# ushariRanasinghe/G2VLM

Hardware: AMD Instinct MI355X
Metric: views/sec (multi-view recon, G2VLM-2B-MoT) (higher is better)
Workload: dtype bf16; 1 GPU; C3: 8-view 518x518 reconstruction, full depth (24 DINO + 28 MoT + 15 decoder blocks), 1 scene per GPU; Lq=10968, Lk=10976, parallelism=replicas x1

## Files before the change

g2vlm_amd/csrc/gemm.hip:

```cpp
#include "common.h"
#include "g2vlm_hip.h"
#include "gemm_internal.h"

namespace {

constexpr int BM = 128, BN = 128, BK = 64;
constexpr int TILE_BYTES = BM * BK * 2;

struct GemmGroup {
  const __bf16* A;
  const __bf16* W;
  const __bf16* bias;
  void* C;
  const void* res;
  const float* gamma;
  int M;
  int tile_start;
};

struct GemmArgs {
  GemmGroup g[2];
  int ngroups, N, K, lda, ldc, ldres, tiles_n, flags, sm, sn, g0_tiles;
};

__device__ __forceinline__ u32x4 ld_chunk(const __bf16* base, int row, int ld, int k, int K) {
  u32x4 z = {0, 0, 0, 0};
  if (k >= K) return z;
  return *reinterpret_cast<const u32x4*>(base + (size_t)row * ld + k);
}

template <int EPI>
__global__ __launch_bounds__(256, 2) void gemm_bf16_kernel(GemmArgs a) {
  __shared__ __attribute__((aligned(16))) char smem[2 * TILE_BYTES];
  char* sA = smem;
  char* sB = smem + TILE_BYTES;

  int bid = blockIdx.x;
  int gi = (a.ngroups > 1 && bid >= a.g[1].tile_start) ? 1 : 0;
  const GemmGroup g = a.g[gi];
  int t = bid - g.tile_start;
  int tm, tn;
  if (a.sm > 1 && gi == 0) {
    const int nt = a.g0_tiles;
    int xcd = t & 7, qn = nt >> 3, rn = nt & 7;
    t = (xcd < rn ? xcd * (qn + 1) : rn * (qn + 1) + (xcd - rn) * qn) + (t >> 3);
    const int tiles_m = (g.M + BM - 1) / BM;
    const int row_sz = a.sm * a.tiles_n;
    int sup_m = t / row_sz, r = t - sup_m * row_sz;
    int h = min(a.sm, tiles_m - sup_m * a.sm);
    int full_w = a.sn * h;
    int sup_n = r / full_w, p = r - sup_n * full_w;
    int width = min(a.sn, a.tiles_n - sup_n * a.sn);
// ... 86 lines not shown
      for (int jp = 0; jp < 2; ++jp) {
        int oc = ((n0 + wn * 64) >> 1) + jp * 16 + cl;
        if (oc >= (N >> 1)) continue;
#pragma unroll
        for (int r = 0; r < 4; ++r) {
          int gm = rbase + i * 16 + r;
          if (gm >= M) continue;
          float gt = bfround(acc[i][2 * jp][r]);
          float up = bfround(acc[i][2 * jp + 1][r]);
          float s = bfround(siluf_fast_(gt));
          C[(size_t)gm * a.ldc + oc] = f2bf(s * up);
        }
      }
    return;
  } else {
#pragma unroll
    for (int j = 0; j < 4; ++j) {
      int gn = n0 + wn * 64 + j * 16 + cl;
      if (gn >= N) continue;
      float bv = g.bias ? bf2f(g.bias[gn]) : 0.f;
      float gam = (EPI == G2V_EPI_RES_F32 && g.gamma) ? g.gamma[gn] : 1.f;
#pragma unroll
      for (int i = 0; i < 4; ++i)
#pragma unroll
        for (int r = 0; r < 4; ++r) {
          int gm = rbase + i * 16 + r;
          if (gm >= M) continue;
          float v = bfround(acc[i][j][r] + bv);
          size_t o = (size_t)gm * a.ldc + gn;
          if constexpr (EPI == G2V_EPI_BF16) {
            reinterpret_cast<__bf16*>(g.C)[o] = f2bf(v);
          } else if constexpr (EPI == G2V_EPI_GELU) {
            reinterpret_cast<__bf16*>(g.C)[o] = f2bf(gelu_erf(v));
          } else if constexpr (EPI == G2V_EPI_QUICKGELU) {
            float u = bfround(1.702f * v);
            float s = bfround(sigmoidf_(u));
            reinterpret_cast<__bf16*>(g.C)[o] = f2bf(v * s);
          } else if constexpr (EPI == G2V_EPI_RES_F32) {
            if (g.gamma) {
              v = __fmul_rn(v, gam);
              if (a.flags & G2V_GEMM_GAMMA_ROUND_BF16) v = bfround(v);
            }
            float rv = g.res ? reinterpret_cast<const float*>(g.res)[(size_t)gm * a.ldres + gn] : 0.f;
            reinterpret_cast<float*>(g.C)[o] = __fadd_rn(rv, v);
          } else if constexpr (EPI == G2V_EPI_RES_BF16) {
            float rv = bf2f(reinterpret_cast<const __bf16*>(g.res)[(size_t)gm * a.ldres + gn]);
            reinterpret_cast<__bf16*>(g.C)[o] = f2bf(rv + v);
          }
        }
    }
  }
}

constexpr int FBK = 16, FLD = 144;

struct GemmF32Args {
  const float* A; const float* W; const float* bias; float* C; const float* res;
  int M, N, K, lda, ldc, ldres, tiles_n, relu;
};

__global__ __launch_bounds__(256, 2) void gemm_f32_kernel(GemmF32Args a) {
  __shared__ __attribute__((aligned(16))) float sA[FBK * FLD];
  __shared__ __attribute__((aligned(16))) float sB[FBK * FLD];
  int tm = blockIdx.x / a.tiles_n, tn = blockIdx.x - tm * a.tiles_n;
  int m0 = tm * 128, n0 = tn * 128;
  const int tid = threadIdx.x, lane = tid & 63, w = tid >> 6, wm = w >> 1, wn = w & 1;
  int srow[2], sk[2], ar[2], br[2];
#pragma unroll
  for (int i = 0; i < 2; ++i) {
    int id = tid + 256 * i;
    srow[i] = id >> 2; sk[i] = (id & 3) * 4;
    ar[i] = min(m0 + srow[i], a.M - 1);
    br[i] = min(n0 + srow[i], a.N - 1);
  }
  f32x4 ra[2], rb[2];
  auto ld4 = [&](const float* base, int row, int ld, int k) -> f32x4 {
    f32x4 v = {0.f, 0.f, 0.f, 0.f};
    const float* p = base + (size_t)row * ld + k;
    if (k + 3 < a.K) v = *reinterpret_cast<const f32x4*>(p);
    else { for (int e = 0; e < 4; ++e) if (k + e < a.K) v[e] = p[e]; }
    return v;
  };
  auto stage_load = [&](int k0) {
#pragma unroll
    for (int i = 0; i < 2; ++i) { ra[i] = ld4(a.A, ar[i], a.lda, k0 + sk[i]); rb[i] = ld4(a.W, br[i], a.K, k0 + sk[i]); }
  };
  auto stage_write = [&]() {
#pragma unroll
    for (int i = 0; i < 2; ++i)
#pragma unroll
      for (int e = 0; e < 4; ++e) { sA[(sk[i] + e) * FLD + srow[i]] = ra[i][e]; sB[(sk[i] + e) * FLD + srow[i]] = rb[i][e]; }
  };
  f32x4 acc[4][4];
#pragma unroll
  for (int i = 0; i < 4; ++i)
#pragma unroll
    for (int j = 0; j < 4; ++j) acc[i][j] = f32x4{0.f, 0.f, 0.f, 0.f};
  const int nk = (a.K + FBK - 1) / FBK;
  stage_load(0); stage_write(); __syncthreads();
  for (int kt = 0; kt < nk; ++kt) {
    if (kt + 1 < nk) stage_load((kt + 1) * FBK);
#pragma unroll
    for (int ks = 0; ks < 4; ++ks) {
      float fa[4], fb[4];
      int kq = ks * 4 + (lane >> 4);
#pragma unroll
      for (int i = 0; i < 4; ++i) {
        fa[i] = sA[kq * FLD + wm * 64 + i * 16 + (lane & 15)];
        fb[i] = sB[kq * FLD + wn * 64 + i * 16 + (lane & 15)];
      }
#pragma unroll
      for (int i = 0; i < 4; ++i)
#pragma unroll
        for (int j = 0; j < 4; ++j) acc[i][j] = __builtin_amdgcn_mfma_f32_16x16x4f32(fa[i], fb[j], acc[i][j], 0, 0, 0);
    }
    __syncthreads();
    if (kt + 1 < nk) { stage_write(); __syncthreads(); }
  }
  const int rbase = m0 + wm * 64 + ((lane >> 4) << 2), cl = lane & 15;
#pragma unroll
  for (int j = 0; j < 4; ++j) {
    int gn = n0 + wn * 64 + j * 16 + cl;
    if (gn >= a.N) continue;
    float bv = a.bias ? a.bias[gn] : 0.f;
#pragma unroll
    for (int i = 0; i < 4; ++i)
#pragma unroll
      for (int r = 0; r < 4; ++r) {
        int gm = rbase + i * 16 + r;
        if (gm >= a.M) continue;
        float v = acc[i][j][r] + bv;
        if (a.relu) v = fmaxf(v, 0.f);
        if (a.res) v = a.res[(size_t)gm * a.ldres + gn] + v;
        a.C[(size_t)gm * a.ldc + gn] = v;
      }
  }
}

template <int EPI>
int launch_bf16(const GemmArgs& a, int total_tiles, hipStream_t s) {
  hipLaunchKernelGGL(gemm_bf16_kernel<EPI>, dim3(total_tiles), dim3(256), 0, s, a);
  G2V_CHECK_LAUNCH();
  return G2V_OK;
}

}

enum { FORM_128 = 1, FORM_BIG = 2, FORM_8P = 3, FORM_4W = 4, FORM_SKINNY = 5 };

static int gemm_route(const g2v_gemm_desc* d, int32_t r[4]) {
  if (!d || d->ngroups < 1 || d->ngroups > 2 || d->N <= 0 || d->K <= 0 || (d->K & 7) || (d->lda & 7)) return G2V_ERR_ARG;
  if (d->epilogue == G2V_EPI_SWIGLU && (d->N & 31)) return G2V_ERR_ARG;
  for (int i = 0; i < d->ngroups; ++i)
    if (d->g[i].M < 0 || !d->g[i].W || !d->g[i].C || (d->g[i].M > 0 && !d->g[i].A)) return G2V_ERR_ARG;
  const bool res_bf16 = d->epilogue == G2V_EPI_RES_BF16;
  r[2] = r[3] = 1;
  const int force = d->flags & (G2V_GEMM_FORCE_SMALL_TILE | G2V_GEMM_FORCE_BIG_TILE | G2V_GEMM_FORCE_8P);
  if (force == 0 && g2v_gemm_skinny_eligible(d)) {
    int M = 0;
    for (int i = 0; i < d->ngroups; ++i) {
      if (res_bf16 && d->g[i].M > 0 && !d->g[i].res) return G2V_ERR_ARG;
      if (d->g[i].M > 0) M = d->g[i].M;
    }
    r[0] = FORM_SKINNY; r[1] = M <= 16 ? 16 : (M <= 32 ? 32 : 64);
    g2v_gemm_skinny_split(d, M, &r[2], &r[3]);
    return G2V_OK;
  }
  if (g2v_gemm_8p_supported(d) && (force == G2V_GEMM_FORCE_8P || (force == 0 && g2v_gemm_8p_preferred(d)))) {
    if (res_bf16)
      for (int i = 0; i < d->ngroups; ++i) if (!d->g[i].res) return G2V_ERR_ARG;
    r[0] = g2v_gemm_8p_four_waves(d) ? FORM_4W : FORM_8P; r[1] = g2v_gemm_8p_height(d);
    return G2V_OK;
  }
  if (!(d->flags & G2V_GEMM_FORCE_SMALL_TILE) && ((d->flags & G2V_GEMM_FORCE_BIG_TILE) ? (d->K % 64 == 0 && d->N % 256 == 0) : g2v_gemm_big_eligible(d))) {
    r[0] = FORM_BIG; r[1] = g2v_gemm_big_height(d);
    return G2V_OK;
  }
  if (res_bf16)
    for (int i = 0; i < d->ngroups; ++i) if (!d->g[i].res) return G2V_ERR_ARG;
  r[0] = FORM_128; r[1] = BM;
  return G2V_OK;
}

extern "C" int g2v_gemm_route(const g2v_gemm_desc* d, int32_t out[4]) {
  if (!out) return G2V_ERR_ARG;
  return gemm_route(d, out);
}

extern "C" int g2v_gemm_bf16(const g2v_gemm_desc* d, void* stream) {
  int32_t r[4];
  const int rc = gemm_route(d, r);
  if (rc != G2V_OK) return rc;
  if (r[0] == FORM_SKINNY) return g2v_gemm_skinny_launch(d, (hipStream_t)stream);
  if (r[0] == FORM_8P || r[0] == FORM_4W) return g2v_gemm_8p_launch(d, (hipStream_t)stream);
  if (r[0] == FORM_BIG) return g2v_gemm_big_launch(d, (hipStream_t)stream);
  GemmArgs a;
  a.ngroups = d->ngroups; a.N = d->N; a.K = d->K; a.lda = d->lda; a.ldc = d->ldc; a.ldres = d->ldres;
  a.tiles_n = (d->N + BN - 1) / BN; a.flags = d->flags;
  int total = 0;
  for (int i = 0; i < 2; ++i) {
    const g2v_gemm_group& s = d->g[i < d->ngroups ? i : 0];
    GemmGroup& g = a.g[i];
    g.A = (const __bf16*)s.A; g.W = (const __bf16*)s.W; g.bias = (const __bf16*)s.bias; g.C = s.C;
    g.res = s.res; g.gamma = (const float*)s.gamma; g.M = s.M; g.tile_start = total;
    if (i < d->ngroups) total += ((s.M + BM - 1) / BM) * a.tiles_n;
  }
  a.sm = 1; a.sn = 1;
  a.sn = a.tiles_n < 12 ? a.tiles_n : 12; a.sm = 96 / a.sn > 1 ? 96 / a.sn : 1;
  if (a.ngroups == 2 && a.g[1].M == 0) a.ngroups = 1;
  if (a.ngroups == 2 && a.g[0].M == 0) { a.g[0] = a.g[1]; a.g[0].tile_start = 0; a.ngroups = 1; }
  if (total == 0) return G2V_OK;
  a.g0_tiles = a.ngroups > 1 ? a.g[1].tile_start : total;
  hipStream_t s = (hipStream_t)stream;
  switch (d->epilogue) {
    case G2V_EPI_BF16: return launch_bf16<G2V_EPI_BF16>(a, total, s);
    case G2V_EPI_GELU: return launch_bf16<G2V_EPI_GELU>(a, total, s);
    case G2V_EPI_QUICKGELU: return launch_bf16<G2V_EPI_QUICKGELU>(a, total, s);
    case G2V_EPI_SWIGLU: return launch_bf16<G2V_EPI_SWIGLU>(a, total, s);
    case G2V_EPI_RES_F32: return launch_bf16<G2V_EPI_RES_F32>(a, total, s);
    case G2V_EPI_RES_BF16: return launch_bf16<G2V_EPI_RES_BF16>(a, total, s);
    default: return G2V_ERR_ARG;
  }
}

extern "C" int g2v_gemm_f32(const void* A, const void* W, const void* bias, void* C, const void* res,
                            int M, int N, int K, int lda, int ldc, int ldres, int relu, void* stream) {
  if (!A || !W || !C || M < 0 || N <= 0 || K <= 0 || (lda & 3) || (K & 3)) return G2V_ERR_ARG;
  if (M == 0) return G2V_OK;
  GemmF32Args a{(const float*)A, (const float*)W, (const float*)bias, (float*)C, (const float*)res,
                M, N, K, lda, ldc, ldres, (N + 127) / 128, relu};
  int tiles = ((M + 127) / 128) * a.tiles_n;
  hipLaunchKernelGGL(gemm_f32_kernel, dim3(tiles), dim3(256), 0, (hipStream_t)stream, a);
  G2V_CHECK_LAUNCH();
  return G2V_OK;
}
```

g2vlm_amd/engine.py:

```python
import math
import os

import torch

from . import hip
from .decode import Decode, KVCache, linear_names, weight_key


def rope2d_tables(D, seq_len, base=100.0):
    inv_freq = 1.0 / (base ** (torch.arange(0, D, 2).float() / D))
    t = torch.arange(seq_len, dtype=inv_freq.dtype)
    freqs = torch.einsum("i,j->ij", t, inv_freq).to(torch.bfloat16)
    freqs = torch.cat((freqs, freqs), dim=-1)
    return freqs.cos(), freqs.sin()


def attn_tile_rows(windows, Hq):
    long_kv = sum(w[3] for w in windows if w[0] == windows[0][0]) >= 2048 and max(w[1] for w in windows) >= 2048
    tall = False
    if not long_kv:
        pad = lambda t: sum((w[1] + t - 1) // t * t for w in windows) / max(1, sum(w[1] for w in windows))
        items = sum((w[1] + 255) // 256 for w in windows) * Hq
        tall = items >= 512 and pad(256) <= 1.12 * pad(128)
    return 256 if (long_kv or tall) else 128
# ... 393 lines not shown
                hp.rope2d(cq, 0, nh, D, cos, sin, pos, P)
                hp.flash_attn(cq, ckv[:, :C], ckv[:, C:], ao, cross_plan, nh, nh, D)
                hp.linear(ao, w[p + "cproj.w"], w[p + "cproj.b"], hp.EPI_RES_F32, out=x, res=x)
                n_mlp = "norm3"
            else:
                n_mlp = "norm2"
            hp.layernorm(x, w[p + n_mlp + ".w"], w[p + n_mlp + ".b"], 1e-6, out=h)
            hp.linear(h, w[p + "mlp.fc1.w"], w[p + "mlp.fc1.b"], hp.EPI_GELU, out=mid)
            hp.linear(mid, w[p + "mlp.fc2.w"], w[p + "mlp.fc2.b"], hp.EPI_RES_F32, out=x, res=x)
        return hp.linear(hp.cast_bf16(x), w[name + ".out.w"], w[name + ".out.b"])

    def decoders_and_heads(self, hidden, context, N, gh, gw, H, W):
        P = gh * gw
        mode = "0" if torch.cuda.is_current_stream_capturing() else os.environ.get("G2V_HEADS_OVERLAP", "2")
        if mode == "0":
            point_hidden = self.decoder("point_decoder", hidden, N, gh, gw)
            camera_hidden = self.decoder("camera_decoder", hidden, N, gh, gw)
            global_hidden = self.decoder("global_points_decoder", hidden, N, gh, gw, context=context)
            points, local, poses, glob = self.heads(point_hidden, camera_hidden, global_hidden, N, H, W)
            return point_hidden, camera_hidden, global_hidden, points, local, poses, glob
        cur = torch.cuda.current_stream()
        side = self.side_stream(cur)
        if mode == "1":
            camera_hidden = self.decoder("camera_decoder", hidden, N, gh, gw)
            side.wait_stream(cur)
            with torch.cuda.stream(side):
                poses = self.camera_poses(camera_hidden, N, P)
            point_hidden = self.decoder("point_decoder", hidden, N, gh, gw)
            side.wait_stream(cur)
            with torch.cuda.stream(side):
                points, local = self.point_maps_local(point_hidden, poses, N, H, W)
            global_hidden = self.decoder("global_points_decoder", hidden, N, gh, gw, context=context)
            cur.wait_stream(side)
            glob = self.point_maps_global(global_hidden, N, H, W)
            return point_hidden, camera_hidden, global_hidden, points, local, poses, glob
        side.wait_stream(cur)
        with torch.cuda.stream(side):
            global_hidden = self.decoder("global_points_decoder", hidden, N, gh, gw, context=context)
            glob = self.point_maps_global(global_hidden, N, H, W)
        camera_hidden = self.decoder("camera_decoder", hidden, N, gh, gw)
        poses = self.camera_poses(camera_hidden, N, P)
        point_hidden = self.decoder("point_decoder", hidden, N, gh, gw)
        points, local = self.point_maps_local(point_hidden, poses, N, H, W)
        cur.wait_stream(side)
        return point_hidden, camera_hidden, global_hidden, points, local, poses, glob

    def side_stream(self, cur):
        key = cur.cuda_stream
        if key not in self._side_streams:
            self._side_streams[key] = torch.cuda.Stream(device=self.dev)
        return self._side_streams[key]

    def conf_head(self, conf_hidden, N, H, W):
        cf = hip.gemm_f32(hip.cast_f32(conf_hidden), self.w["conf_head.w"], self.w["conf_head.b"])
        return hip.pixel_shuffle(cf, N, H, W, 1, self.patch)

    def camera_poses(self, camera_hidden, N, P):
        w, hp = self.w, hip
        feat = hp.cast_f32(camera_hidden)
        for i in range(2):
            t = hp.gemm_f32(feat, w[f"cam.res{i}.1.w"], w[f"cam.res{i}.1.b"], relu=True)
            t = hp.gemm_f32(t, w[f"cam.res{i}.2.w"], w[f"cam.res{i}.2.b"], relu=True)
            feat = hp.gemm_f32(t, w[f"cam.res{i}.3.w"], w[f"cam.res{i}.3.b"], relu=True, res=feat)
        return hp.camera_tail(feat, N, P, w["cam.mlp0.w"], w["cam.mlp0.b"], w["cam.mlp1.w"], w["cam.mlp1.b"],
                              w["cam.fc_t.w"], w["cam.fc_t.b"], w["cam.fc_rot.w"], w["cam.fc_rot.b"])

    def point_maps(self, point_hidden, global_hidden, poses, N, H, W):
        points, local = self.point_maps_local(point_hidden, poses, N, H, W)
        return points, local, self.point_maps_global(global_hidden, N, H, W)

    def point_maps_local(self, point_hidden, poses, N, H, W):
        w, hp = self.w, hip
        pf = hp.gemm_f32(hp.cast_f32(point_hidden), w["point_head.w"], w["point_head.b"])
        local, points = hp.pts_epilogue(pf, N, H, W, 1, poses, patch=self.patch)
        return points, local

    def point_maps_global(self, global_hidden, N, H, W):
        w, hp = self.w, hip
        gf = hp.gemm_f32(hp.cast_f32(global_hidden), w["global_point_head.w"], w["global_point_head.b"])
        glob, _ = hp.pts_epilogue(gf, N, H, W, 0, patch=self.patch)
        return glob

    def heads(self, point_hidden, camera_hidden, global_hidden, N, H, W):
        poses = self.camera_poses(camera_hidden, N, (H // self.patch) * (W // self.patch))
        points, local, glob = self.point_maps(point_hidden, global_hidden, poses, N, H, W)
        return points, local, poses, glob

    def vit_forward(self, pixel_values, grid_thw, cos, sin, num_layers=None, n_images=1):
        w, hp = self.w, hip
        V = self.dims["vit"]
        C, nh = V["embed"], V["heads"]
        D = C // nh
        T = pixel_values.shape[0]
        t, gh, gw = grid_thw
        t = t * n_images
        assert pixel_values.shape[1] == w["vit.patch.w"].shape[1] and T == t * gh * gw
        x = hp.linear(pixel_values if pixel_values.dtype == torch.bfloat16 else hp.cast_bf16(pixel_values), w["vit.patch.w"], None)
        plan = self.plan(tuple((i * gh * gw, gh * gw, i * gh * gw, gh * gw, False) for i in range(t)), nh)
        h = torch.empty((T, C), dtype=torch.bfloat16, device=self.dev)
        qkv = torch.empty((T, 3 * C), dtype=torch.bfloat16, device=self.dev)
        ao = torch.empty((T, C), dtype=torch.bfloat16, device=self.dev)
        mid = torch.empty((T, int(C * V["mlp_ratio"])), dtype=torch.bfloat16, device=self.dev)
        for i in range(V["depth"] if num_layers is None else num_layers):
            p = f"V{i}."
            hp.layernorm(x, w[p + "norm1.w"], w[p + "norm1.b"], 1e-6, out=h)
            hp.linear(h, w[p + "attn.qkv.w"], w[p + "attn.qkv.b"], out=qkv)
            hp.rope_vision(qkv, 2 * nh, D, cos, sin)
            hp.flash_attn(qkv[:, :C], qkv[:, C:2 * C], qkv[:, 2 * C:], ao, plan, nh, nh, D)
            hp.linear(ao, w[p + "attn.proj.w"], w[p + "attn.proj.b"], hp.EPI_RES_BF16, out=x, res=x)
            hp.layernorm(x, w[p + "norm2.w"], w[p + "norm2.b"], 1e-6, out=h)
            hp.linear(h, w[p + "mlp.fc1.w"], w[p + "mlp.fc1.b"], hp.EPI_QUICKGELU, out=mid)
            hp.linear(mid, w[p + "mlp.fc2.w"], w[p + "mlp.fc2.b"], hp.EPI_RES_BF16, out=x, res=x)
        hp.layernorm(x, w["vit.ln_q.w"], w["vit.ln_q.b"], 1e-6, out=h)
        m = hp.linear(h.view(T // 4, 4 * C), w["vit.m0.w"], w["vit.m0.b"], hp.EPI_GELU)
        return hp.linear(m, w["vit.m2.w"], w["vit.m2.b"])
```

g2vlm_amd/hip.py:

```python
import ctypes as C
import os
import threading

import torch

_HERE = os.path.dirname(os.path.abspath(__file__))
LIB_PATH = os.environ.get("G2V_LIB_PATH") or os.path.join(_HERE, "lib", "libg2vlm_hip.so")

EPI_BF16, EPI_GELU, EPI_QUICKGELU, EPI_SWIGLU, EPI_RES_F32, EPI_RES_BF16 = range(6)
GAMMA_ROUND_BF16 = 1
FORCE_SMALL_TILE = 2
SUPERTILE = 4
FORCE_BIG_TILE = 8
FORCE_8P = 16
P8_H192, P8_H128, P8_H256, P8_TWO_BARRIER, P8_H288, P8_H224, P8_H160 = 128, 256, 512, 1024, 4096, 8192, 16384
P8_PIPELINED = 32768
P8_FOUR_WAVES = 65536
P8_EIGHT_WAVES = 131072
P8_NO_ROW_SKIP = 262144
F32, BF16 = 0, 1
NO_CAUSAL = 2 ** 30
_DEBUG_GEMM_FLAGS = int(os.environ.get("G2V_GEMM_FLAGS", "0"))


class GemmGroup(C.Structure):
    _fields_ = [("A", C.c_void_p), ("W", C.c_void_p), ("bias", C.c_void_p), ("C", C.c_void_p),
                ("res", C.c_void_p), ("gamma", C.c_void_p), ("M", C.c_int32), ("_pad", C.c_int32)]


class GemmDesc(C.Structure):
    _fields_ = [("g", GemmGroup * 2), ("ngroups", C.c_int32), ("N", C.c_int32), ("K", C.c_int32),
                ("lda", C.c_int32), ("ldc", C.c_int32), ("ldres", C.c_int32), ("epilogue", C.c_int32),
                ("flags", C.c_int32), ("workspace", C.c_void_p), ("workspace_bytes", C.c_int64)]


_P, _I, _F, _L = C.c_void_p, C.c_int, C.c_float, C.c_int64
_SIGS = {
    "g2v_version": ([], C.c_int),
    "g2v_arch": ([], C.c_char_p),
    "g2v_gemm_bf16": ([C.POINTER(GemmDesc), _P], C.c_int),
    "g2v_gemm_route": ([C.POINTER(GemmDesc), C.POINTER(C.c_int32 * 4)], C.c_int),
    "g2v_gemm_f32": ([_P, _P, _P, _P, _P, _I, _I, _I, _I, _I, _I, _I, _P], C.c_int),
    "g2v_layernorm": ([_P, _I, _I, _P, _P, _F, _P, _I, _I, _I, _I, _P], C.c_int),
    "g2v_rmsnorm": ([_P, _I, _P, _P, _I, _F, _P, _I, _I, _I, _I, _P], C.c_int),
    "g2v_mrope_table": ([_P, _I, _P, _P, _P, _P], C.c_int),
    "g2v_qknorm_mrope_cache": ([_P, _I, _I, _I, _P, _P, _P, _P, _I, _F, _I, _P, _P, _P, _P, _P, _P, _P], C.c_int),
    "g2v_flash_attn": ([_P, _I, _P, _I, _P, _I, _P, _I, _P, _I, _I, _I, _I, _F, _P, _P, _I, _P, _I, _I, _P, _P], C.c_int),
    "g2v_flash_attn_workspace": ([_I], C.c_int64),
    "g2v_debug_attn_form": ([_I], C.c_int),
    "g2v_rope2d": ([_P, _I, _I, _I, _I, _I, _P, _P, _P, _I, _P], C.c_int),
    "g2v_rope_vision": ([_P, _I, _I, _I, _I, _P, _P, _P], C.c_int),
    "g2v_im2col14": ([_P, _I, _I, _I, _P, _I, _P], C.c_int),
    "g2v_dino_preprocess": ([_P, _I, _I, _I, _I, C.POINTER(C.c_float), C.POINTER(C.c_float), _P, _P, _P], C.c_int),
    "g2v_dino_assemble": ([_P, _P, _P, _P, _P, _I, _I, _I, _P], C.c_int),
    "g2v_im2col_patch": ([_P, _I, _I, _I, _I, _P, _I, _P], C.c_int),
    "g2v_qwen_patchify_u8": ([_P, _I, _I, _I, C.POINTER(C.c_float), C.POINTER(C.c_float), _P, _I, _P], C.c_int),
    "g2v_vit_assemble": ([_P, _P, _P, _P, _I, _I, _I, _I, _P], C.c_int),
    "g2v_gather_rows_f32": ([_P, _I, _P, _P, _I, _I, _I, _P], C.c_int),
    "g2v_scatter_rows_f32": ([_P, _I, _P, _P, _I, _I, _I, _P], C.c_int),
    "g2v_cast_f32_bf16": ([_P, _P, _L, _P], C.c_int),
    "g2v_cast_bf16_f32": ([_P, _P, _L, _P], C.c_int),
    "g2v_pts_epilogue": ([_P, _I, _I, _I, _I, _P, _P, _P, _P], C.c_int),
    "g2v_pixel_shuffle14": ([_P, _I, _I, _I, _I, _P, _P], C.c_int),
    "g2v_lanczos_resize_u8": ([_P, _I, _I, _I, _P, _I, _I, _P, _P, _P, _I, _P, _P, _I, _P], C.c_int),
    "g2v_pts_epilogue_ps": ([_P, _I, _I, _I, _I, _I, _P, _P, _P, _P], C.c_int),
    "g2v_pixel_shuffle": ([_P, _I, _I, _I, _I, _I, _P, _P], C.c_int),
    "g2v_camera_tail": ([_P, _I, _I, _P, _P, _P, _P, _P, _P, _P, _P, _P, _P], C.c_int),
    "g2v_argmax_bf16": ([_P, _I, _P, _P, _P], C.c_int),
    "g2v_gemv_bf16": ([_P, _P, _P, _P, _P, _I, _I, _P], C.c_int),
    "g2v_decode_attn_workspace": ([_I, _I], C.c_int64),
    "g2v_gemv_rmsnorm_bf16": ([_P, _P, _F, _P, _P, _P, _I, _I, _P], C.c_int),
    "g2v_gemv_swiglu_bf16": ([_P, _P, _P, _I, _I, _P], C.c_int),
    "g2v_gemv_rmsnorm_swiglu_bf16": ([_P, _P, _F, _P, _P, _I, _I, _P], C.c_int),
    "g2v_decode_attn": ([_P, _P, _P, _P, _I, _I, _I, _F, _P, _P], C.c_int),
    "g2v_swiglu_bf16": ([_P, _P, _I, _P], C.c_int),
    "g2v_decode_attn_dyn": ([_P, _P, _P, _P, _P, _I, _I, _I, _F, _P, _P], C.c_int),
    "g2v_decode_advance": ([_P, _P, _P, _P], C.c_int),
    "g2v_decode_attn_batch": ([_P, _P, _P, _P, _P, _I, _L, _I, _I, _I, _F, _P, _P], C.c_int),
    "g2v_decode_advance_batch": ([_P, _P, _P, _I, _P], C.c_int),
    "g2v_decode_attn_fused": ([_P, _P, _P, _F, _I, _P, _P, _P, _P, _P, _P, _I, _L, _I, _I, _I, _F, _P, _P], C.c_int),
    "g2v_argmax_rows_bf16": ([_P, _I, _I, _L, _P, _P, _P], C.c_int),
    "g2v_gemv_pg": ([_P, _P, _F, _P, _P, _P, _P, _I, _I, _I, _P], C.c_int),
    "g2v_gemv_pg_batch": ([_P, _P, _F, _P, _P, _P, _P, _I, _I, _I, _I, _P], C.c_int),
    "g2v_decode_attn_pg_workspace": ([_I, _I, _I], C.c_int64),
    "g2v_decode_attn_pg": ([_P, _P, _P, _F, _I, _P, _P, _P, _P, _P, _P, _I, _L, _I, _I, _I, _F, _P, _P], C.c_int),
    "g2v_sample_rows_bf16": ([_P, _I, _I, _L, _P, _P, _P, _P], C.c_int),
    "g2v_decode_attn_shared_workspace": ([_I, _I, _I, _I, _I], C.c_int64),
    "g2v_decode_attn_shared": ([_P, _P, _P, _F, _I, _P, _P, _P, _P, _I, _P, _P, _P, _I, _L, _I, _I, _I, _F, _P, _P, _P], C.c_int),
    "g2v_gemv_pg_fp8": ([_P, _P, _F, _P, _P, _P, _P, _P, _I, _I, _I, _P], C.c_int),
    "g2v_gemv_pg_batch_fp8": ([_P, _P, _F, _P, _P, _P, _P, _P, _I, _I, _I, _I, _P], C.c_int),
    "g2v_gemv_pg_route": ([_I, _I, _I, _I, _I, _I, C.POINTER(C.c_int32 * 4)], C.c_int),
    "g2v_kv_quant_e4m3": ([_P, _L, _I, _P, _P, _P], C.c_int),
    "g2v_kv_dequant_e4m3": ([_P, _P, _L, _I, _P, _P], C.c_int),
    "g2v_decode_attn_pg_kv8": ([_P, _P, _P, _F, _I, _P, _P, _P, _P, _P, _P, _P, _P, _I, _L, _I, _I, _I, _F, _P, _P], C.c_int),
    "g2v_logprob_rows_workspace": ([_I, _I], C.c_int64),
# ... 86 lines not shown
    if ws is None:
        ws = _gemm_ws[key] = torch.zeros(GEMM_WS_WORDS, dtype=torch.int32, device=device)
    return ws


def gemm_bf16(groups, N, K, epilogue, out_ld, lda=None, ldres=0, flags=0, ws=None):
    _ck(lib().g2v_gemm_bf16(C.byref(_gemm_desc(groups, N, K, epilogue, out_ld, lda, ldres, flags, ws)), _stream()), "g2v_gemm_bf16")


GEMM_FORMS = {1: "128x128", 2: "big", 3: "8p", 4: "4w", 5: "skinny"}


def gemm_route(groups, N, K, epilogue, out_ld, lda=None, ldres=0, flags=0, ws=None):
    out = (C.c_int32 * 4)()
    _ck(lib().g2v_gemm_route(C.byref(_gemm_desc(groups, N, K, epilogue, out_ld, lda, ldres, flags, ws)), C.byref(out)),
        "g2v_gemm_route")
    return GEMM_FORMS[out[0]], out[1], out[2], out[3]


def _gemm_desc(groups, N, K, epilogue, out_ld, lda, ldres, flags, ws):
    d = GemmDesc()
    flags |= _DEBUG_GEMM_FLAGS
    d.ngroups, d.N, d.K, d.epilogue, d.flags = len(groups), N, K, epilogue, flags
    d.lda = lda if lda is not None else K
    d.ldc, d.ldres = out_ld, ldres
    if max(int(g["M"]) for g in groups) <= 64:
        if ws is None:
            ws = _gemm_workspace(groups[0]["A"].device)
        d.workspace, d.workspace_bytes = ws.data_ptr(), ws.numel() * ws.element_size()
    for i, g in enumerate(groups):
        gg = d.g[i]
        gg.A, gg.W, gg.bias, gg.C = _p(g["A"]), _p(g["W"]), _p(g.get("bias")), _p(g["C"])
        gg.res, gg.gamma, gg.M = _p(g.get("res")), _p(g.get("gamma")), int(g["M"])
    return d


def linear(x, w, bias=None, epilogue=EPI_BF16, out=None, res=None, gamma=None, flags=0, ws=None):
    M, K = x.shape
    N = w.shape[0]
    n_out = N // 2 if epilogue == EPI_SWIGLU else N
    if out is None:
        dt = torch.float32 if epilogue == EPI_RES_F32 else torch.bfloat16
        out = torch.empty((M, n_out), dtype=dt, device=x.device)
    gemm_bf16([dict(A=x, W=w, bias=bias, C=out, res=res, gamma=gamma, M=M)], N, K, epilogue,
              out_ld=_rowmajor(out), lda=_rowmajor(x), ldres=_rowmajor(res) if res is not None else 0, flags=flags, ws=ws)
    return out


def gemm_f32(x, w, bias=None, relu=False, res=None, out=None):
    M, K = x.shape
    N = w.shape[0]
    if out is None:
        out = torch.empty((M, N), dtype=torch.float32, device=x.device)
    _ck(lib().g2v_gemm_f32(_p(x), _p(w), _p(bias), _p(out), _p(res), M, N, K, _rowmajor(x), _rowmajor(out),
                           _rowmajor(res) if res is not None else 0, int(relu), _stream()), "g2v_gemm_f32")
    return out


def _dt(t):
    return BF16 if t.dtype == torch.bfloat16 else F32


def layernorm(x, w, b, eps, out_dtype=torch.bfloat16, out=None):
    M, Cc = x.shape
    if out is None:
        out = torch.empty((M, Cc), dtype=out_dtype, device=x.device)
    _ck(lib().g2v_layernorm(_p(x), _dt(x), _rowmajor(x), _p(w), _p(b), eps, _p(out), _dt(out), _rowmajor(out), M, Cc,
                            _stream()), "g2v_layernorm")
    return out


def rmsnorm(x, w_lo, w_hi, split, eps, out_dtype=torch.bfloat16, out=None):
    M, Cc = x.shape
    if out is None:
        out = torch.empty((M, Cc), dtype=out_dtype, device=x.device)
    _ck(lib().g2v_rmsnorm(_p(x), _rowmajor(x), _p(w_lo), _p(w_hi), int(split), eps, _p(out), _dt(out), _rowmajor(out),
                          M, Cc, _stream()), "g2v_rmsnorm")
    return out


def mrope_table(pos_i32, inv_freq):
    L = pos_i32.shape[1]
    cos = torch.empty((L, 128), dtype=torch.float32, device=pos_i32.device)
    sin = torch.empty_like(cos)
    _ck(lib().g2v_mrope_table(_p(pos_i32), L, _p(inv_freq), _p(cos), _p(sin), _stream()), "g2v_mrope_table")
    return cos, sin


def qknorm_mrope_cache(qkv, Hq, Hkv, qw_lo, qw_hi, kw_lo, kw_hi, split, eps, und_rounding, cos, sin, q_out, k_cache,
                       v_cache, kv_rows):
    L = qkv.shape[0]
    _ck(lib().g2v_qknorm_mrope_cache(_p(qkv), L, Hq, Hkv, _p(qw_lo), _p(qw_hi), _p(kw_lo), _p(kw_hi), int(split), eps,
                                     int(und_rounding), _p(cos), _p(sin), _p(q_out), _p(k_cache), _p(v_cache),
                                     _p(kv_rows), _stream()), "g2v_qknorm_mrope_cache")


class AttnSeg(C.Structure):
    _fields_ = [("desc", C.c_int32), ("head", C.c_int32), ("kt0", C.c_int32), ("kt1", C.c_int32), ("slot", C.c_int32),
                ("_pad", C.c_int32 * 3)]


class AttnPlan:

    def __init__(self, tiles, n_tiles, phases, comb, n_comb, n_slots, tile_rows, device):
        self.tiles, self.n_tiles, self.phases = tiles, n_tiles, phases
        self.comb, self.n_comb, self.n_slots, self.tile_rows = comb, n_comb, n_slots, tile_rows
        self.n_blocks = max((p[2] for p in phases), default=0)
        self.n_split = n_comb
        self.ws_words = max(4, int(lib().g2v_flash_attn_workspace(n_slots)) // 4)
# ... 530 lines not shown
```

include/g2vlm_hip.h:

```cpp
#ifndef G2VLM_HIP_H
#define G2VLM_HIP_H
#include <stdint.h>
#ifdef __cplusplus
extern "C" {
#endif

int g2v_version(void);
const char* g2v_arch(void);

enum {
  G2V_EPI_BF16 = 0,
  G2V_EPI_GELU = 1,
  G2V_EPI_QUICKGELU = 2,
  G2V_EPI_SWIGLU = 3,
  G2V_EPI_RES_F32 = 4,
  G2V_EPI_RES_BF16 = 5
};
#define G2V_GEMM_GAMMA_ROUND_BF16 1
#define G2V_GEMM_SUPERTILE 4
#define G2V_GEMM_FORCE_BIG_TILE 8
#define G2V_GEMM_FORCE_8P 16
#define G2V_GEMM_8P_H192 128
#define G2V_GEMM_8P_H128 256
#define G2V_GEMM_8P_H256 512
#define G2V_GEMM_8P_TWO_BARRIER 1024
#define G2V_GEMM_8P_H288 4096
#define G2V_GEMM_8P_H224 8192
#define G2V_GEMM_8P_H160 16384
#define G2V_GEMM_8P_PIPELINED 32768
#define G2V_GEMM_8P_FOUR_WAVES 65536
#define G2V_GEMM_8P_NO_ROW_SKIP 262144
#define G2V_GEMM_8P_EIGHT_WAVES 131072
#define G2V_GEMM_FORCE_SMALL_TILE 2

typedef struct {
  const void* A;
  const void* W;
  const void* bias;
  void* C;
  const void* res;
  const void* gamma;
  int32_t M;
  int32_t _pad;
} g2v_gemm_group;

typedef struct {
  g2v_gemm_group g[2];
  int32_t ngroups, N, K, lda, ldc, ldres, epilogue, flags;
  void* workspace;
  int64_t workspace_bytes;
} g2v_gemm_desc;

int g2v_gemm_bf16(const g2v_gemm_desc* desc, void* stream);
int g2v_gemm_route(const g2v_gemm_desc* desc, int32_t out[4]);

int g2v_gemm_f32(const void* A, const void* W, const void* bias, void* C, const void* res,
                 int M, int N, int K, int lda, int ldc, int ldres, int relu, void* stream);

#define G2V_F32 0
#define G2V_BF16 1
int g2v_layernorm(const void* x, int x_dtype, int ldx, const void* w, const void* b, float eps,
                  void* out, int out_dtype, int ldo, int M, int C, void* stream);
int g2v_rmsnorm(const void* x, int ldx, const void* w_lo, const void* w_hi, int split, float eps,
                void* out, int out_dtype, int ldo, int M, int C, void* stream);

int g2v_mrope_table(const void* pos, int L, const void* inv_freq , void* cos, void* sin, void* stream);
int g2v_qknorm_mrope_cache(const void* qkv, int L, int Hq, int Hkv,
                           const void* qw_lo, const void* qw_hi, const void* kw_lo, const void* kw_hi,
                           int split, float eps, int und_rounding, const void* cos, const void* sin,
                           void* q_out, void* k_cache, void* v_cache, const void* kv_rows, void* stream);

typedef struct {
  int32_t q0, q_rows;
  int32_t k0, k_len;
  int32_t causal_shift;
  int32_t q_win0;
  int32_t _pad[2];
} g2v_attn_tile;

typedef struct {
  int32_t desc;
  int32_t head;
  int32_t kt0, kt1;
  int32_t slot;
  int32_t _pad[3];
} g2v_attn_seg;
int64_t g2v_flash_attn_workspace(int n_slots);
int g2v_debug_attn_form(int form);
int g2v_flash_attn(const void* q, int ldq, const void* k, int ldk, const void* v, int ldv,
                   void* o, int ldo, const g2v_attn_tile* tiles, int n_tiles,
                   int Hq, int Hkv, int D, float scale,
                   const g2v_attn_seg* segs, const int32_t* seg_ptr, int n_blocks, const int32_t* comb, int n_comb,
                   int tile_rows, void* workspace, void* stream);

int g2v_rope2d(void* x, int ld, int M, int col0, int n_heads, int D, const void* cos, const void* sin,
               const void* pos, int P, void* stream);

int g2v_rope_vision(void* x, int ld, int M, int n_heads, int D, const void* cos, const void* sin, void* stream);

int g2v_dino_preprocess(const void* in, int in_is_u8, int N, int H, int W, const float* mean3, const float* std3, void* norm,
                        void* orig, void* stream);

int g2v_lanczos_resize_u8(const void* src, int N, int Hin, int Win, void* dst, int Hout, int Wout, void* tmp,
                          const void* bounds_h, const void* kk_h, int ksize_h,
                          const void* bounds_v, const void* kk_v, int ksize_v, void* stream);
int g2v_im2col14(const void* img, int N, int H, int W, void* out, int Kpad, void* stream);
int g2v_dino_assemble(const void* patch, const void* cls, const void* regs, const void* pos,
                      void* x, int N, int P, int C, void* stream);

int g2v_im2col_patch(const void* img, int N, int H, int W, int patch, void* out, int Kpad, void* stream);
// ... 96 lines not shown
```

Before: 115.7 views/s.

## Rewrite f32 head GEMM with adaptive row tiles and fused bf16 input widening

Replaces the fixed 128x128 fp32 MFMA GEMM with a templated kernel. It picks the M-tile height from the CU count so the head projections fill the GPU, double-buffers the K-tiles in dynamic LDS and interleaves the LDS writes with the MFMAs. It also remaps block indices across XCDs and vectorises the epilogue stores. A bf16-input variant widens activations inside the kernel, so the conf, point and global heads no longer need a separate cast_f32 pass. In exchange there are 28 template instantiations, much more LDS per block, and a per-kernel static attribute setup.

Measured after the change: 116.3 views/s (median of 6 runs). About the same (+0.5%).

```diff
diff --git a/g2vlm_amd/csrc/gemm.hip b/g2vlm_amd/csrc/gemm.hip
--- a/g2vlm_amd/csrc/gemm.hip
+++ b/g2vlm_amd/csrc/gemm.hip
@@ -1,3 +1,5 @@
+#include <type_traits>
+
 #include "common.h"
 #include "g2vlm_hip.h"
 #include "gemm_internal.h"
@@ -190,88 +192,225 @@
   }
 }
 
-constexpr int FBK = 16, FLD = 144;
+constexpr int FBK = 32, FLD = 34, FBN = 128, FTM_MAX = 14;
 
 struct GemmF32Args {
-  const float* A; const float* W; const float* bias; float* C; const float* res;
-  int M, N, K, lda, ldc, ldres, tiles_n, relu;
+  const void* A; const float* W; const float* bias; float* C; const float* res;
+  int M, N, K, lda, ldc, ldres, tiles_n, relu, vec, total;
 };
 
-__global__ __launch_bounds__(256, 2) void gemm_f32_kernel(GemmF32Args a) {
-  __shared__ __attribute__((aligned(16))) float sA[FBK * FLD];
-  __shared__ __attribute__((aligned(16))) float sB[FBK * FLD];
-  int tm = blockIdx.x / a.tiles_n, tn = blockIdx.x - tm * a.tiles_n;
-  int m0 = tm * 128, n0 = tn * 128;
-  const int tid = threadIdx.x, lane = tid & 63, w = tid >> 6, wm = w >> 1, wn = w & 1;
-  int srow[2], sk[2], ar[2], br[2];
-#pragma unroll
-  for (int i = 0; i < 2; ++i) {
-    int id = tid + 256 * i;
-    srow[i] = id >> 2; sk[i] = (id & 3) * 4;
-    ar[i] = min(m0 + srow[i], a.M - 1);
-    br[i] = min(n0 + srow[i], a.N - 1);
-  }
-  f32x4 ra[2], rb[2];
-  auto ld4 = [&](const float* base, int row, int ld, int k) -> f32x4 {
-    f32x4 v = {0.f, 0.f, 0.f, 0.f};
-    const float* p = base + (size_t)row * ld + k;
-    if (k + 3 < a.K) v = *reinterpret_cast<const f32x4*>(p);
-    else { for (int e = 0; e < 4; ++e) if (k + e < a.K) v[e] = p[e]; }
-    return v;
-  };
+typedef __attribute__((ext_vector_type(2))) float f32x2;
+
+template <int TM, bool A16>
+__global__ __launch_bounds__(256) void gemm_f32_kernel(GemmF32Args a) {
+  extern __shared__ __attribute__((aligned(16))) float fsm[];
+  constexpr int BMF = TM * 16, STAGE = (BMF + FBN) * FLD;
+  constexpr int NA = (TM + 1) / 2, NB = 4;
+  using araw = typename std::conditional<A16, u32x2, f32x4>::type;
+
+  int t = blockIdx.x;
+  {
+    const int nt = a.total, xcd = t & 7, qn = nt >> 3, rn = nt & 7;
+    t = (xcd < rn ? xcd * (qn + 1) : rn * (qn + 1) + (xcd - rn) * qn) + (t >> 3);
+  }
+  const int tmi = t / a.tiles_n, tn = t - tmi * a.tiles_n;
+  const int m0 = tmi * BMF, n0 = tn * FBN;
+  const int tid = threadIdx.x, lane = tid & 63, wn = __builtin_amdgcn_readfirstlane(tid >> 6);
+  const int M = a.M, N = a.N, K = a.K;
+
+  const int sc = (tid & 7) * 4;
+  const char* pa[NA];
+  const float* pb[NB];
+  int wa[NA], wb[NB];
+#pragma unroll
+  for (int i = 0; i < NA; ++i) {
+    const int row = (tid + 256 * i) >> 3;
+    const size_t o = (size_t)min(m0 + row, M - 1) * a.lda + sc;
+    pa[i] = reinterpret_cast<const char*>(a.A) + o * (A16 ? 2 : 4);
+    wa[i] = row * FLD + sc;
+  }
+#pragma unroll
+  for (int i = 0; i < NB; ++i) {
+    const int row = (tid + 256 * i) >> 3;
+    pb[i] = a.W + (size_t)min(n0 + row, N - 1) * K + sc;
+    wb[i] = (BMF + row) * FLD + sc;
+  }
+  araw ra[NA];
+  f32x4 rb[NB];
   auto stage_load = [&](int k0) {
-#pragma unroll
-    for (int i = 0; i < 2; ++i) { ra[i] = ld4(a.A, ar[i], a.lda, k0 + sk[i]); rb[i] = ld4(a.W, br[i], a.K, k0 + sk[i]); }
-  };
-  auto stage_write = [&]() {
-#pragma unroll
-    for (int i = 0; i < 2; ++i)
-#pragma unroll
-      for (int e = 0; e < 4; ++e) { sA[(sk[i] + e) * FLD + srow[i]] = ra[i][e]; sB[(sk[i] + e) * FLD + srow[i]] = rb[i][e]; }
-  };
-  f32x4 acc[4][4];
-#pragma unroll
-  for (int i = 0; i < 4; ++i)
-#pragma unroll
-    for (int j = 0; j < 4; ++j) acc[i][j] = f32x4{0.f, 0.f, 0.f, 0.f};
-  const int nk = (a.K + FBK - 1) / FBK;
-  stage_load(0); stage_write(); __syncthreads();
-  for (int kt = 0; kt < nk; ++kt) {
-    if (kt + 1 < nk) stage_load((kt + 1) * FBK);
-#pragma unroll
-    for (int ks = 0; ks < 4; ++ks) {
-      float fa[4], fb[4];
-      int kq = ks * 4 + (lane >> 4);
-#pragma unroll
-      for (int i = 0; i < 4; ++i) {
-        fa[i] = sA[kq * FLD + wm * 64 + i * 16 + (lane & 15)];
-        fb[i] = sB[kq * FLD + wn * 64 + i * 16 + (lane & 15)];
+    const bool in = k0 + sc < K;
+#pragma unroll
+    for (int i = 0; i < NA; ++i) {
+      araw z = {};
+      if (in && (2 * i + 1 < TM || tid < 128)) z = *reinterpret_cast<const araw*>(pa[i] + (size_t)k0 * (A16 ? 2 : 4));
+      ra[i] = z;
+    }
+#pragma unroll
+    for (int i = 0; i < NB; ++i) {
+      f32x4 z = {0.f, 0.f, 0.f, 0.f};
+      if (in) z = *reinterpret_cast<const f32x4*>(pb[i] + k0);
+      rb[i] = z;
+    }
+  };
+  auto put = [&](float* p, f32x4 v) {
+    *reinterpret_cast<f32x2*>(p) = f32x2{v[0], v[1]};
+    *reinterpret_cast<f32x2*>(p + 2) = f32x2{v[2], v[3]};
+  };
+  auto widen = [&](araw r) -> f32x4 {
+    if constexpr (A16) return f32x4{bits2f_lo(r[0]), bits2f_hi(r[0]), bits2f_lo(r[1]), bits2f_hi(r[1])};
+    else return r;
+  };
+  auto stage_write = [&](float* st, int part) {
+#pragma unroll
+    for (int i = 0; i < NA; ++i)
+      if ((i & 3) == part && (2 * i + 1 < TM || tid < 128)) put(st + wa[i], widen(ra[i]));
+#pragma unroll
+    for (int i = 0; i < NB; ++i)
+      if (((NA + i) & 3) == part) put(st + wb[i], rb[i]);
+  };
+
+  const int nj = min(2, max(0, (N - (n0 + wn * 32) + 15) >> 4));
+  f32x4 acc[TM][2];
+#pragma unroll
+  for (int i = 0; i < TM; ++i) acc[i][0] = acc[i][1] = f32x4{0.f, 0.f, 0.f, 0.f};
+  const int aoff = (lane & 15) * FLD + (lane >> 4);
+  const int boff = (BMF + wn * 32 + (lane & 15)) * FLD + (lane >> 4);
+
+  auto k_tile = [&](auto njc, const float* cur, float* nxt) {
+    constexpr int NJ = decltype(njc)::value;
+    float fa[2][TM], fb[2][NJ > 0 ? NJ : 1];
+    auto frags = [&](int ks) {
+#pragma unroll
+      for (int j = 0; j < NJ; ++j) fb[ks & 1][j] = cur[boff + j * 16 * FLD + ks * 4];
+#pragma unroll
+      for (int i = 0; i < TM; ++i) fa[ks & 1][i] = cur[aoff + i * 16 * FLD + ks * 4];
+    };
+    if constexpr (NJ > 0) frags(0);
+#pragma unroll
+    for (int ks = 0; ks < FBK / 4; ++ks) {
+      if constexpr (NJ > 0) {
+        if (ks + 1 < FBK / 4) frags(ks + 1);
+#pragma unroll
+        for (int i = 0; i < TM; ++i)
+#pragma unroll
+          for (int j = 0; j < NJ; ++j)
+            acc[i][j] = __builtin_amdgcn_mfma_f32_16x16x4f32(fb[ks & 1][j], fa[ks & 1][i], acc[i][j], 0, 0, 0);
       }
-#pragma unroll
-      for (int i = 0; i < 4; ++i)
-#pragma unroll
-        for (int j = 0; j < 4; ++j) acc[i][j] = __builtin_amdgcn_mfma_f32_16x16x4f32(fa[i], fb[j], acc[i][j], 0, 0, 0);
-    }
-    __syncthreads();
-    if (kt + 1 < nk) { stage_write(); __syncthreads(); }
-  }
-  const int rbase = m0 + wm * 64 + ((lane >> 4) << 2), cl = lane & 15;
-#pragma unroll
-  for (int j = 0; j < 4; ++j) {
-    int gn = n0 + wn * 64 + j * 16 + cl;
-    if (gn >= a.N) continue;
-    float bv = a.bias ? a.bias[gn] : 0.f;
-#pragma unroll
-    for (int i = 0; i < 4; ++i)
-#pragma unroll
-      for (int r = 0; r < 4; ++r) {
-        int gm = rbase + i * 16 + r;
-        if (gm >= a.M) continue;
-        float v = acc[i][j][r] + bv;
-        if (a.relu) v = fmaxf(v, 0.f);
-        if (a.res) v = a.res[(size_t)gm * a.ldres + gn] + v;
-        a.C[(size_t)gm * a.ldc + gn] = v;
+      if (ks >= 3 && ks < 7) stage_write(nxt, ks - 3);
+      __builtin_amdgcn_sched_barrier(0);
+    }
+  };
+
+  const int nk = (K + FBK - 1) / FBK;
+  stage_load(0);
+#pragma unroll
+  for (int p = 0; p < 4; ++p) stage_write(fsm, p);
+  __syncthreads();
+  auto k_loop = [&](auto njc) {
+    for (int kt = 0; kt < nk; ++kt) {
+      stage_load((kt + 1) * FBK);
+      k_tile(njc, fsm + (kt & 1) * STAGE, fsm + ((kt + 1) & 1) * STAGE);
+      __syncthreads();
+    }
+  };
+  if (nj == 2) k_loop(std::integral_constant<int, 2>{});
+  else if (nj == 1) k_loop(std::integral_constant<int, 1>{});
+  else k_loop(std::integral_constant<int, 0>{});
+
+  const int cq = n0 + wn * 32 + ((lane >> 4) << 2);
+  float bv[2][4];
+#pragma unroll
+  for (int j = 0; j < 2; ++j)
+#pragma unroll
+    for (int r = 0; r < 4; ++r) {
+      const int gn = cq + j * 16 + r;
+      bv[j][r] = (a.bias && gn < N) ? a.bias[gn] : 0.f;
+    }
+#pragma unroll
+  for (int i = 0; i < TM; ++i) {
+    const int gm = m0 + i * 16 + (lane & 15);
+    if (gm >= M) continue;
+#pragma unroll
+    for (int j = 0; j < 2; ++j) {
+      const int gn = cq + j * 16;
+      if (gn >= N) continue;
+      float* cp = a.C + (size_t)gm * a.ldc + gn;
+      const float* rp = a.res ? a.res + (size_t)gm * a.ldres + gn : nullptr;
+      if (a.vec && gn + 3 < N) {
+        f32x4 rv = {0.f, 0.f, 0.f, 0.f}, o;
+        if (rp) rv = *reinterpret_cast<const f32x4*>(rp);
+#pragma unroll
+        for (int r = 0; r < 4; ++r) {
+          float v = acc[i][j][r] + bv[j][r];
+          if (a.relu) v = fmaxf(v, 0.f);
+          if (rp) v = rv[r] + v;
+          o[r] = v;
+        }
+        *reinterpret_cast<f32x4*>(cp) = o;
+      } else {
+#pragma unroll
+        for (int r = 0; r < 4; ++r) {
+          if (gn + r >= N) continue;
+          float v = acc[i][j][r] + bv[j][r];
+          if (a.relu) v = fmaxf(v, 0.f);
+          if (rp) v = rp[r] + v;
+          cp[r] = v;
+        }
       }
+    }
+  }
+}
+
+int g_f32_rows = 0;
+
+int f32_tile_rows(int M, int tiles_n) {
+  static int n_cu = 0;
+  if (n_cu == 0) {
+    int dev = 0;
+    hipDeviceProp_t prop;
+    n_cu = (hipGetDevice(&dev) == hipSuccess && hipGetDeviceProperties(&prop, dev) == hipSuccess && prop.multiProcessorCount > 0)
+               ? prop.multiProcessorCount : 256;
+  }
+  const int slots = n_cu / tiles_n > 1 ? n_cu / tiles_n : 1;
+  for (int rounds = 1;; ++rounds) {
+    const long per = 16L * slots * rounds;
+    const int tm = (int)((M + per - 1) / per);
+    if (tm <= FTM_MAX) return tm < 1 ? 1 : tm;
+  }
+}
+
+template <int TM, bool A16>
+int launch_f32_tm(const GemmF32Args& a, hipStream_t s) {
+  constexpr int LDS = 2 * (TM * 16 + FBN) * FLD * 4;
+  static bool attr_set = false;
+  if (!attr_set) {
+    if (hipFuncSetAttribute(reinterpret_cast<const void*>(gemm_f32_kernel<TM, A16>), hipFuncAttributeMaxDynamicSharedMemorySize,
+                            LDS) != hipSuccess) return G2V_ERR_LAUNCH;
+    attr_set = true;
+  }
+  GemmF32Args b = a;
+  b.total = ((a.M + TM * 16 - 1) / (TM * 16)) * a.tiles_n;
+  hipLaunchKernelGGL((gemm_f32_kernel<TM, A16>), dim3(b.total), dim3(256), LDS, s, b);
+  G2V_CHECK_LAUNCH();
+  return G2V_OK;
+}
+
+template <bool A16>
+int launch_f32(const void* A, const void* W, const void* bias, void* C, const void* res, int M, int N, int K, int lda, int ldc,
+               int ldres, int relu, hipStream_t s) {
+  if (!A || !W || !C || M < 0 || N <= 0 || K <= 0 || (lda & 3) || (K & 3)) return G2V_ERR_ARG;
+  if (M == 0) return G2V_OK;
+  auto al16 = [](const void* p) { return (reinterpret_cast<uintptr_t>(p) & 15) == 0; };
+  GemmF32Args a{A, (const float*)W, (const float*)bias, (float*)C, (const float*)res, M, N, K, lda, ldc, ldres,
+                (N + FBN - 1) / FBN, relu, 0, 0};
+  a.vec = al16(C) && !(ldc & 3) && (!res || (al16(res) && !(ldres & 3)));
+  const int tm = g_f32_rows ? g_f32_rows : f32_tile_rows(M, a.tiles_n);
+  switch (tm) {
+#define F32_TM(T) case T: return launch_f32_tm<T, A16>(a, s);
+    F32_TM(1) F32_TM(2) F32_TM(3) F32_TM(4) F32_TM(5) F32_TM(6) F32_TM(7) F32_TM(8) F32_TM(9) F32_TM(10) F32_TM(11) F32_TM(12)
+    F32_TM(13) F32_TM(14)
+#undef F32_TM
+    default: return G2V_ERR_ARG;
   }
 }
 
@@ -363,12 +502,16 @@
 
 extern "C" int g2v_gemm_f32(const void* A, const void* W, const void* bias, void* C, const void* res,
                             int M, int N, int K, int lda, int ldc, int ldres, int relu, void* stream) {
-  if (!A || !W || !C || M < 0 || N <= 0 || K <= 0 || (lda & 3) || (K & 3)) return G2V_ERR_ARG;
-  if (M == 0) return G2V_OK;
-  GemmF32Args a{(const float*)A, (const float*)W, (const float*)bias, (float*)C, (const float*)res,
-                M, N, K, lda, ldc, ldres, (N + 127) / 128, relu};
-  int tiles = ((M + 127) / 128) * a.tiles_n;
-  hipLaunchKernelGGL(gemm_f32_kernel, dim3(tiles), dim3(256), 0, (hipStream_t)stream, a);
-  G2V_CHECK_LAUNCH();
+  return launch_f32<false>(A, W, bias, C, res, M, N, K, lda, ldc, ldres, relu, (hipStream_t)stream);
+}
+
+extern "C" int g2v_gemm_f32_a16(const void* A, const void* W, const void* bias, void* C, const void* res,
+                                int M, int N, int K, int lda, int ldc, int ldres, int relu, void* stream) {
+  return launch_f32<true>(A, W, bias, C, res, M, N, K, lda, ldc, ldres, relu, (hipStream_t)stream);
+}
+
+extern "C" int g2v_debug_gemm_f32_rows(int rows) {
+  if (rows < 0 || rows > 16 * FTM_MAX || (rows & 15)) return G2V_ERR_ARG;
+  g_f32_rows = rows / 16;
   return G2V_OK;
 }
diff --git a/g2vlm_amd/engine.py b/g2vlm_amd/engine.py
--- a/g2vlm_amd/engine.py
+++ b/g2vlm_amd/engine.py
@@ -469,7 +469,7 @@
         return self._side_streams[key]
 
     def conf_head(self, conf_hidden, N, H, W):
-        cf = hip.gemm_f32(hip.cast_f32(conf_hidden), self.w["conf_head.w"], self.w["conf_head.b"])
+        cf = hip.gemm_f32(conf_hidden, self.w["conf_head.w"], self.w["conf_head.b"])
         return hip.pixel_shuffle(cf, N, H, W, 1, self.patch)
 
     def camera_poses(self, camera_hidden, N, P):
@@ -488,13 +488,13 @@
 
     def point_maps_local(self, point_hidden, poses, N, H, W):
         w, hp = self.w, hip
-        pf = hp.gemm_f32(hp.cast_f32(point_hidden), w["point_head.w"], w["point_head.b"])
+        pf = hp.gemm_f32(point_hidden, w["point_head.w"], w["point_head.b"])
         local, points = hp.pts_epilogue(pf, N, H, W, 1, poses, patch=self.patch)
         return points, local
 
     def point_maps_global(self, global_hidden, N, H, W):
         w, hp = self.w, hip
-        gf = hp.gemm_f32(hp.cast_f32(global_hidden), w["global_point_head.w"], w["global_point_head.b"])
+        gf = hp.gemm_f32(global_hidden, w["global_point_head.w"], w["global_point_head.b"])
         glob, _ = hp.pts_epilogue(gf, N, H, W, 0, patch=self.patch)
         return glob
 
diff --git a/g2vlm_amd/hip.py b/g2vlm_amd/hip.py
--- a/g2vlm_amd/hip.py
+++ b/g2vlm_amd/hip.py
@@ -41,6 +41,8 @@
     "g2v_gemm_bf16": ([C.POINTER(GemmDesc), _P], C.c_int),
     "g2v_gemm_route": ([C.POINTER(GemmDesc), C.POINTER(C.c_int32 * 4)], C.c_int),
     "g2v_gemm_f32": ([_P, _P, _P, _P, _P, _I, _I, _I, _I, _I, _I, _I, _P], C.c_int),
+    "g2v_gemm_f32_a16": ([_P, _P, _P, _P, _P, _I, _I, _I, _I, _I, _I, _I, _P], C.c_int),
+    "g2v_debug_gemm_f32_rows": ([_I], C.c_int),
     "g2v_layernorm": ([_P, _I, _I, _P, _P, _F, _P, _I, _I, _I, _I, _P], C.c_int),
     "g2v_rmsnorm": ([_P, _I, _P, _P, _I, _F, _P, _I, _I, _I, _I, _P], C.c_int),
     "g2v_mrope_table": ([_P, _I, _P, _P, _P, _P], C.c_int),
@@ -233,9 +235,18 @@
     N = w.shape[0]
     if out is None:
         out = torch.empty((M, N), dtype=torch.float32, device=x.device)
-    _ck(lib().g2v_gemm_f32(_p(x), _p(w), _p(bias), _p(out), _p(res), M, N, K, _rowmajor(x), _rowmajor(out),
-                           _rowmajor(res) if res is not None else 0, int(relu), _stream()), "g2v_gemm_f32")
-    return out
+    if x.dtype == torch.bfloat16:
+        fn, what = lib().g2v_gemm_f32_a16, "g2v_gemm_f32_a16"
+    else:
+        assert x.dtype == torch.float32, x.dtype
+        fn, what = lib().g2v_gemm_f32, "g2v_gemm_f32"
+    _ck(fn(_p(x), _p(w), _p(bias), _p(out), _p(res), M, N, K, _rowmajor(x), _rowmajor(out),
+           _rowmajor(res) if res is not None else 0, int(relu), _stream()), what)
+    return out
+
+
+def debug_gemm_f32_rows(rows):
+    _ck(lib().g2v_debug_gemm_f32_rows(int(rows)), "g2v_debug_gemm_f32_rows")
 
 
 def _dt(t):
diff --git a/include/g2vlm_hip.h b/include/g2vlm_hip.h
--- a/include/g2vlm_hip.h
+++ b/include/g2vlm_hip.h
@@ -56,6 +56,9 @@
 
 int g2v_gemm_f32(const void* A, const void* W, const void* bias, void* C, const void* res,
                  int M, int N, int K, int lda, int ldc, int ldres, int relu, void* stream);
+int g2v_gemm_f32_a16(const void* A, const void* W, const void* bias, void* C, const void* res,
+                     int M, int N, int K, int lda, int ldc, int ldres, int relu, void* stream);
+int g2v_debug_gemm_f32_rows(int rows);
 
 #define G2V_F32 0
 #define G2V_BF16 1
```
